# google-research/frame-interpolation

Measured on NVIDIA H100. Metric: interpolated_frames_per_sec_1080p, higher is better.
Workload: dtype f16x2-split (activations/weights as fp16 hi+lo planes; fp32 accumulate)

## Files before the change

### frame_interpolation_b200/csrc/film_conv3x3_tc.cu

```cuda
#include <cuda.h>
#include <cuda_runtime.h>
#include <stdint.h>

#include <type_traits>

#include "film_conv.h"
#include "film_tc_ptx.cuh"

namespace film {
namespace {
using namespace tc;

constexpr int kConsumers = 256;
constexpr int kThreads = kConsumers + 128;
__host__ __device__ constexpr int a_plane_bytes(int kc, int th, int tw) { return (th + 2) * tw * kc * 2; }
__host__ __device__ constexpr int a_stage_bytes(int kc, int th, int tw) { return 2 * a_plane_bytes(kc, th, tw); }
constexpr int kHaloW = 10;
__host__ __device__ constexpr int halo_box_bytes(int kc, int th) { return (th + 2) * kHaloW * kc * 2; }
__host__ __device__ constexpr int halo_plane_bytes(int kc, int th) { return (halo_box_bytes(kc, th) + 1023) & ~1023; }
__host__ __device__ constexpr int a_stage_bytes_h(int kc, int th, int tw, int halo, int planes = 2) {
  return planes * (halo ? halo_plane_bytes(kc, th) : a_plane_bytes(kc, th, tw));
}
constexpr int kMaxRing = 8;
constexpr int kSmemLimit = 227 * 1024;
constexpr int kBarBytes = 8 * (4 * kMaxRing + 4);
constexpr int kFixedBytes = kBarBytes + 16 + 512 * 4  + 64  + 1024  + 64;
constexpr int kHeadW3 = 64 * 32 * 4, kHeadMisc = 512;
constexpr int kHeadBytes = kHeadW3 + kHeadMisc;
constexpr int kPxnStageWg = 64 * 64 * 2;
constexpr int kPxnStageBytes = 2 * kPxnStageWg;
inline int epi_scratch_bytes(int epi_mode, int pxn) { return epi_mode == 3 ? kHeadBytes : pxn ? kPxnStageBytes : 0; }

__host__ __device__ inline int w_tap_bytes(int bn, int kc, int planes = 2) { return bn * kc * 2 * planes; }

template <int BN, int KC, bool kPartial, bool kHalo, bool kOne, bool kRes, bool kPxN = false>
__global__ void __launch_bounds__(kThreads, 1) k_conv3x3_tc(const ConvProblem* __restrict__ prob) {
  static_assert(!kPxN || ((BN == 64 || BN == 128) && KC == 64), "pixels on N: one or two M = 64 weight tiles, 64-channel chunks");
  extern __shared__ uint8_t smem_raw[];
  constexpr bool one = kOne;
  const int planes = one ? 1 : 2;
  constexpr int kWPlane = BN * KC * 2;
  const int kWTap = kWPlane * planes;
  const int kTileH = prob->tile_h, kTileW = prob->tile_w;
  constexpr int kHaloTileH = kPxN ? 32 : 16;
  constexpr int kHaloBox = halo_box_bytes(KC, kHaloTileH), kHaloPlane = halo_plane_bytes(KC, kHaloTileH);
  constexpr bool halo = kHalo;
  const int kAPlane = halo ? kHaloPlane : a_plane_bytes(KC, kTileH, kTileW);
  const int kAStage = planes * kAPlane;
  const int kRowStep = kTileW * KC * 2;
  constexpr bool kFused = BN <= 128 && !kPxN;
  constexpr int kMh = kPxN ? BN / 64 : 1;
  constexpr int kAccRegs = kPxN ? 64 * kMh : (kFused ? 2 * BN : BN) / 2;
  constexpr int kWgPx = kPxN ? 128 : 64;

  const int NA = prob->v2_na, NW = prob->v2_nw;
  const bool resident = prob->v2_resident != 0;
  const int nsrc = prob->nsrc;
  const int tiles_x = prob->tiles_x, tiles_per_img = prob->tiles_y * prob->tiles_x;
  const int cout = prob->cout;
  const int n_nt = (cout + BN - 1) / BN;
  const int ntiles = prob->B * tiles_per_img * n_nt;
  constexpr int kStageTaps = kHalo ? 9 : 3;
  constexpr bool kPacked = kPartial && kPxN;
  const int part_lo = prob->v2_part_lo, part_hi = prob->v2_part_hi;
  int nab = 0;
  for (int s = 0; s < nsrc; ++s) nab += prob->src[s].nchunk * (kHalo ? 1 : 3);
  const int nkb = nab * kStageTaps - (kPacked ? (part_hi - part_lo) * (kStageTaps - kStageTaps / 3) : 0);

  const FastDiv div_nt(n_nt, ntiles), div_img(tiles_per_img, ntiles), div_tx(tiles_x, ntiles);
  const bool pair = prob->pair != 0;
  const int rank = pair ? (int)cluster_ctarank() : 0;
  const int nsp = prob->B * tiles_per_img;
  const int nwork = pair ? ((nsp + 1) / 2) * n_nt : ntiles;
  const int w_first = pair ? (int)blockIdx.x >> 1 : (int)blockIdx.x, w_step = pair ? (int)gridDim.x >> 1 : (int)gridDim.x;
  auto decode = [&](int work, int& sp, int& nti) {
    div_nt.divmod(work, sp, nti);
    if (pair) sp = 2 * sp + rank;
  };

  const uint32_t raw = smem_u32(smem_raw);
  const uint32_t base = (raw + 1023u) & ~1023u;
  uint8_t* gen_base = smem_raw + (base - raw);
// ... 83 lines not shown
        for (int ch = 0; ch < nchunk; ++ch) {
          const int nst = halo ? 1 : 3;
          for (int dx = 0; dx < nst; ++dx, ++ab) {
            const int st = ra.stage;
            mbar_wait(tail + 8u * (kMaxRing + st), ra.phase ^ 1u);
            if (elect_one()) {
              const uint32_t sa = a_base + st * kAStage, bar = tail + 8u * st;
              mbar_expect_tx(bar, halo ? (uint32_t)(planes * kHaloBox) : (uint32_t)kAStage);
              tma_load_4d(sa, tm_hi, bar, c_off + ch * KC, x0 + dx - 1, y0 - 1, bs);
              if (!one) tma_load_4d(sa + kAPlane, tm_lo, bar, c_off + ch * KC, x0 + dx - 1, y0 - 1, bs);
            }
            __syncwarp();
            ra.advance(NA);
            if (!resident) {
              const bool packed = kPacked && ab >= part_lo && ab < part_hi;
              const int nblk = packed ? kStageTaps / 3 : kStageTaps;
              for (int t = 0; t < nblk; ++t, ++kb) {
                const int ws = rw.stage;
                mbar_wait(tail + 8u * (3 * kMaxRing + ws), rw.phase ^ 1u);
                if (elect_one()) {
                  const uint32_t sw = w_base + ws * kWTap, bar = tail + 8u * (2 * kMaxRing + ws);
                  mbar_expect_tx(bar, kWTap);
                  if (pair) {
                    const uint32_t hoff = (uint32_t)(rank * (kWPlane / 2));
                    tma_load_2d_mc(sw + hoff, &prob->tm_w_hi_half, bar, kb * KC, n0 + rank * (BN / 2), 3);
                    if (!one) tma_load_2d_mc(sw + kWPlane + hoff, &prob->tm_w_lo_half, bar, kb * KC, n0 + rank * (BN / 2), 3);
                  } else {
                    tma_load_2d(sw, tm_w_hi, bar, kb * KC, n0);
                    if (!one) tma_load_2d(sw + kWPlane, tm_w_lo, bar, kb * KC, n0);
                  }
                }
// ... 45 lines not shown

  if (resident) mbar_wait(tail + 8u * (2 * kMaxRing), 0);
  const bool is_leader = (threadIdx.x & 127) == 0;
  const uint32_t w_empty_peer = pair ? map_to_cta(tail + 8u * (3 * kMaxRing), (uint32_t)(rank ^ 1)) : 0u;
  auto release_w = [&](int slot) {
    mbar_arrive(tail + 8u * (3 * kMaxRing + slot));
    if (pair) mbar_arrive_cluster(w_empty_peer + 8u * slot);
  };
  {
    constexpr int kWTapC = kWPlane * (kOne ? 1 : 2);
    constexpr uint32_t kPx = KC * 2;
    const uint32_t a_row0 = kHalo ? (uint32_t)(wg * (kWgPx / 8) * kHaloW) * kPx : (uint32_t)(wg * kWgPx) * kPx;
    const uint32_t sbo = kHalo ? kHaloW * kPx : 8 * kPx;
    RingPos ra, rw;
    float acc[kAccRegs];
    auto pxn_mma = [&](uint64_t w_hi, uint64_t w_lo, uint64_t a_hi, uint64_t a_lo, uint32_t accf) {
#pragma unroll
      for (int h = 0; h < kMh; ++h) {
        const uint64_t wh = (uint64_t)(h * (64 * KC * 2) >> 4);
        wgmma<128>(acc + 64 * h, w_hi + wh, a_hi, accf);
        if constexpr (!kOne) {
          wgmma<128>(acc + 64 * h, w_lo + wh, a_hi, 1u);
          wgmma<128>(acc + 64 * h, w_hi + wh, a_lo, 1u);
        }
      }
    };
    for (int tile = w_first; tile < nwork; tile += w_step) {
      int kb = 0;
      int rel_a = -1, rel_w = -1;
      auto retire = [&](int next_a, int next_w) {
        wgmma_commit();
        wgmma_wait<1>();
        if (is_leader) {
          if (rel_a >= 0) mbar_arrive(tail + 8u * (kMaxRing + rel_a));
          if (rel_w >= 0) release_w(rel_w);
        }
        rel_a = next_a;
        rel_w = next_w;
      };
      auto stage = [&](auto ksteps_c, auto tpb_c) {
        constexpr int kSteps = decltype(ksteps_c)::value, kTpb = decltype(tpb_c)::value;
        constexpr int kBlocks = kStageTaps / kTpb;
        const int st = ra.stage;
        mbar_wait(tail + 8u * st, ra.phase);
        const uint32_t sa = a_base + st * kAStage + a_row0;
        const uint32_t lo_off = (uint32_t)(kHalo ? kHaloPlane : kAPlane);
        if constexpr (kRes) {
          const uint64_t a0 = make_desc_sbo<KC>(sa, sbo);
          const uint64_t lo_delta = (uint64_t)(lo_off >> 4);
          const uint64_t row_delta = (uint64_t)(kRowStep >> 4);
          const uint64_t w0 = make_desc_kc<KC>(w_base + kb * kWTapC);
          const uint32_t first = (kb == 0) ? 0u : 1u;
          wgmma_fence();
#pragma unroll
          for (int t = 0; t < kStageTaps; ++t) {
            const uint64_t a_hi = a0 + (kHalo ? (uint64_t)((((t % 3) * kHaloW + t / 3) * kPx) >> 4) : (uint64_t)t * row_delta);
            const uint64_t a_lo = a_hi + lo_delta;
            const uint64_t w_hi = w0 + (uint64_t)(((t / kTpb) * kWTapC + (t % kTpb) * kSteps * 32) >> 4);
            const uint64_t w_lo = w_hi + (uint64_t)(kWPlane >> 4);
#pragma unroll
            for (int k = 0; k < kSteps; ++k) {
              const uint64_t adv = (uint64_t)(k * 32 >> 4);
              const uint32_t accf = (t == 0 && k == 0) ? first : 1u;
              if constexpr (kPxN) {
                pxn_mma(w_hi + adv, w_lo + adv, a_hi + adv, a_lo + adv, accf);
              } else if constexpr (kOne) {
                wgmma<BN>(acc, a_hi + adv, w_hi + adv, accf);
              } else if constexpr (kFused) {
                wgmma<BN>(acc, a_hi + adv, w_hi + adv, accf);
                wgmma<BN>(acc + BN / 2, a_hi + adv, w_lo + adv, accf);
                wgmma<BN>(acc, a_lo + adv, w_hi + adv, 1u);
              } else {
                wgmma<BN>(acc, a_lo + adv, w_hi + adv, accf);
                wgmma<BN>(acc, a_hi + adv, w_lo + adv, 1u);
                wgmma<BN>(acc, a_hi + adv, w_hi + adv, 1u);
              }
            }
          }
// ... 2 lines not shown
        } else {
          for (int blk = 0; blk < kBlocks; ++blk, ++kb) {
            uint32_t sw;
            int ws = -1;
            if (resident) {
              sw = w_base + kb * kWTap;
            } else {
              ws = rw.stage;
              mbar_wait(tail + 8u * (2 * kMaxRing + ws), rw.phase);
              sw = w_base + ws * kWTap;
            }
            const uint32_t first = (kb == 0) ? 0u : 1u;
            wgmma_fence();
#pragma unroll
            for (int u = 0; u < kTpb; ++u) {
              const int t = blk * kTpb + u;
              const uint32_t off = kHalo ? (uint32_t)((t % 3) * kHaloW + t / 3) * kPx : (uint32_t)(t * kRowStep);
              const uint64_t a_hi = make_desc_sbo<KC>(sa + off, sbo);
              const uint64_t a_lo = make_desc_sbo<KC>(sa + lo_off + off, sbo);
              const uint64_t wk = (uint64_t)((u * kSteps * 32) >> 4);
              const uint64_t w_hi = make_desc_kc<KC>(sw) + wk, w_lo = make_desc_kc<KC>(sw + kWPlane) + wk;
#pragma unroll
              for (int k = 0; k < kSteps; ++k) {
                const uint64_t adv = (uint64_t)(k * 32 >> 4);
                const uint32_t accf = (u == 0 && k == 0) ? first : 1u;
                if constexpr (kPxN) {
                  pxn_mma(w_hi + adv, w_lo + adv, a_hi + adv, a_lo + adv, accf);
                } else if constexpr (kOne) {
                  wgmma<BN>(acc, a_hi + adv, w_hi + adv, accf);
                } else if constexpr (kFused) {
                  wgmma<BN>(acc, a_hi + adv, w_hi + adv, accf);
// ... 22 lines not shown
        for (int ab = 0; ab < nab; ++ab) stage(Full{}, One{});
      }
      wgmma_wait<0>();
      if (is_leader) {
        if (rel_a >= 0) mbar_arrive(tail + 8u * (kMaxRing + rel_a));
        if (rel_w >= 0) release_w(rel_w);
      }
      acc_fence<kAccRegs>(acc);

      int sp, nti, b, rem, ty, tx;
      decode(tile, sp, nti);
      div_img.divmod(sp, b, rem);
      div_tx.divmod(rem, ty, tx);
      const int n0 = nti * BN;
      const bool live = sp < nsp;
      if constexpr (kPxN) {
        const int c0 = 16 * (warp & 3) + (lane >> 2);
#pragma unroll
        for (int m = 0; m < kMh; ++m) {
          const float bias0 = bias_smem[n0 + 64 * m + c0], bias1 = bias_smem[n0 + 64 * m + c0 + 8];
#pragma unroll
          for (int i = 64 * m; i < 64 * m + 64; ++i) {
            const float f = acc[i] + ((i & 2) ? bias1 : bias0);
            acc[i] = act ? leaky(f) : f;
          }
        }
        const int y_wg = ty * kTileH + 16 * wg, x_t = tx * kTileW;
        if (do_pool) {
          const int px = x_t + 2 * q;
#pragma unroll
          for (int j = 0; j < 16; j += 2) {
// ... 189 lines not shown
            uint32_t hi, lo;
            split_pack2((a[0][0] + a[1][0]) * 0.25f, (a[0][1] + a[1][1]) * 0.25f, hi, lo);
            *reinterpret_cast<uint32_t*>(pool_hi + ppix * pool_C + n0 + c) = hi;
            *reinterpret_cast<uint32_t*>(pool_lo + ppix * pool_C + n0 + c) = lo;
          }
        }
      }
    }
  }
  leave();
}

int smem_bytes_for(const ConvProblem& h, int bn) {
  const int nkb = h.ktot / h.kchunk;
  const int planes = h.passes == 1 ? 1 : 2;
  const int w = h.v2_resident ? nkb * w_tap_bytes(bn, h.kchunk, planes) : h.v2_nw * w_tap_bytes(bn, h.kchunk, planes);
  return h.v2_na * a_stage_bytes_h(h.kchunk, h.tile_h, h.tile_w, h.halo, planes) + w + kFixedBytes +
         epi_scratch_bytes(h.epi_mode, h.pxn);
}

}

int conv_tc_block_n(int cout);

namespace {
bool ring_depths(int kc, int tile_h, int tile_w, int halo, int planes, int bn, int cout, int ktot, int epi_mode, int pxn,
                 int& resident, int& na, int& nw) {
  const int wtap = w_tap_bytes(bn, kc, planes);
  const int w_all = (ktot / kc) * wtap;
  const int kLimit = kSmemLimit - epi_scratch_bytes(epi_mode, pxn);
  const int kAStage = a_stage_bytes_h(kc, tile_h, tile_w, halo, planes);
  if (cout <= bn && w_all + 2 * kAStage + kFixedBytes <= kLimit) {
    resident = 1;
    const int n = (kLimit - kFixedBytes - w_all) / kAStage;
    const int n_max = halo ? 3 : 6;
    na = n > n_max ? n_max : n;
    nw = 1;
    return true;
  }
  resident = 0;
  na = halo ? 2 : (bn >= 128 ? 2 : 3);
  int n = (kLimit - kFixedBytes - na * kAStage) / wtap;
  if (n < 2 && na > 2) {
    na = 2;
    n = (kLimit - kFixedBytes - na * kAStage) / wtap;
// ... 16 lines not shown
    if (!ring_depths(kc, c[0], c[1], 0, passes == 1 ? 1 : 2, bn, cout, ktot, epi_mode, 0, res, na, nw)) continue;
    const long tiles = (long)B * ((H + c[0] - 1) / c[0]) * ((W + c[1] - 1) / c[1]) * n_nt;
    const long waves = (tiles + num_sms - 1) / num_sms;
    const double cost = (double)waves * (c[0] + 2.0) / c[0] * (1.0 + 1e-3 * (c[1] / 8));
    if (cost < best) {
      best = cost;
      tile_h = c[0];
      tile_w = c[1];
    }
  }
}

bool conv3x3_tc_plan(ConvProblem& h, int num_sms) {
  const int bn = h.bn;
  const int planes = h.passes == 1 ? 1 : 2;
  const int wtap = w_tap_bytes(bn, h.kchunk, planes);
  const int w_all = (h.ktot / h.kchunk) * wtap;
  const bool can_resident = h.cout <= bn;
  const int kLimit = kSmemLimit - epi_scratch_bytes(h.epi_mode, h.pxn);
  if (h.halo && (h.tile_h != (h.pxn ? 32 : 16) || h.tile_w != 8 ||
                 (can_resident && w_all + 2 * a_stage_bytes_h(h.kchunk, h.tile_h, h.tile_w, 0, planes) + kFixedBytes <= kLimit &&
                  w_all + 2 * a_stage_bytes_h(h.kchunk, h.tile_h, h.tile_w, 1, planes) + kFixedBytes > kLimit)))
    h.halo = 0;
  bool ok = ring_depths(h.kchunk, h.tile_h, h.tile_w, h.halo, planes, bn, h.cout, h.ktot, h.epi_mode, h.pxn,
                        h.v2_resident, h.v2_na, h.v2_nw);
  if (!ok && h.halo) {
    h.halo = 0;
    ok = ring_depths(h.kchunk, h.tile_h, h.tile_w, 0, planes, bn, h.cout, h.ktot, h.epi_mode, h.pxn, h.v2_resident,
                     h.v2_na, h.v2_nw);
  }
  const int nsp = h.B * h.tiles_y * h.tiles_x, n_nt = (h.cout + bn - 1) / bn;
  if (h.pair) {
    const int nwork = (nsp + 1) / 2 * n_nt, nclu = num_sms / 2;
    h.v2_grid = 2 * (nwork < nclu ? nwork : nclu);
  } else {
    h.v2_grid = nsp * n_nt < num_sms ? nsp * n_nt : num_sms;
  }
  return ok;
}

template <int BN, int KC, bool kPxN = false>
struct Variants {
  static constexpr void (*kFn[16])(const ConvProblem*) = {
      k_conv3x3_tc<BN, KC, false, false, false, false, kPxN>, k_conv3x3_tc<BN, KC, false, false, false, true, kPxN>,
      k_conv3x3_tc<BN, KC, false, false, true, false, kPxN>,  k_conv3x3_tc<BN, KC, false, false, true, true, kPxN>,
      k_conv3x3_tc<BN, KC, false, true, false, false, kPxN>,  k_conv3x3_tc<BN, KC, false, true, false, true, kPxN>,
      k_conv3x3_tc<BN, KC, false, true, true, false, kPxN>,   k_conv3x3_tc<BN, KC, false, true, true, true, kPxN>,
      k_conv3x3_tc<BN, KC, true, false, false, false, kPxN>,  k_conv3x3_tc<BN, KC, true, false, false, true, kPxN>,
      k_conv3x3_tc<BN, KC, true, false, true, false, kPxN>,   k_conv3x3_tc<BN, KC, true, false, true, true, kPxN>,
      k_conv3x3_tc<BN, KC, true, true, false, false, kPxN>,   k_conv3x3_tc<BN, KC, true, true, false, true, kPxN>,
      k_conv3x3_tc<BN, KC, true, true, true, false, kPxN>,    k_conv3x3_tc<BN, KC, true, true, true, true, kPxN>};
  static cudaError_t configure() {
    for (auto fn : kFn) {
      const cudaError_t e = cudaFuncSetAttribute(fn, cudaFuncAttributeMaxDynamicSharedMemorySize, kSmemLimit);
      if (e != cudaSuccess) return e;
    }
    return cudaSuccess;
  }
  static cudaError_t launch(const ConvProblem* d_prob, const ConvProblem& h, cudaStream_t st) {
    if (h.v2_na < 2 || (!h.v2_resident && h.v2_nw < 2)) return cudaErrorInvalidValue;
    if (kPxN && (h.pair || h.tile_h != 32 || h.tile_w != 8 || h.epi_mode != 0)) return cudaErrorInvalidValue;
    const bool partial = h.v2_part_hi > h.v2_part_lo;
    const int idx = (partial ? 8 : 0) | (h.halo ? 4 : 0) | (h.passes == 1 ? 2 : 0) | (h.v2_resident && h.straight ? 1 : 0);
    if (!h.pair) {
      kFn[idx]<<<h.v2_grid, kThreads, smem_bytes_for(h, BN), st>>>(d_prob);
      return cudaGetLastError();
    }
    cudaLaunchConfig_t cfg = {};
    cudaLaunchAttribute attr[1];
    attr[0].id = cudaLaunchAttributeClusterDimension;
    attr[0].val.clusterDim.x = 2;
    attr[0].val.clusterDim.y = 1;
    attr[0].val.clusterDim.z = 1;
    cfg.gridDim = dim3(h.v2_grid);
    cfg.blockDim = dim3(kThreads);
    cfg.dynamicSmemBytes = smem_bytes_for(h, BN);
    cfg.stream = st;
    cfg.attrs = attr;
// ... 1 lines not shown
    return cudaLaunchKernelEx(&cfg, kFn[idx], d_prob);
  }
};

cudaError_t conv3x3_tc_configure() {
  cudaError_t e;
#define FILM_CFG(BN, KC)                        \
  e = Variants<BN, KC>::configure();            \
  if (e != cudaSuccess) return e;
  FILM_CFG(32, 64) FILM_CFG(64, 64) FILM_CFG(128, 64) FILM_CFG(256, 64) FILM_CFG(32, 32) FILM_CFG(64, 32)
#undef FILM_CFG
  e = Variants<64, 64, true>::configure();
  if (e != cudaSuccess) return e;
  e = Variants<128, 64, true>::configure();
  if (e != cudaSuccess) return e;
  return cudaSuccess;
}

cudaError_t launch_conv3x3_tc(const ConvProblem* d_prob, const ConvProblem& h, cudaStream_t st) {
  const int bn = h.bn;
  if (h.kchunk == 32) {
    if (bn == 32) return Variants<32, 32>::launch(d_prob, h, st);
    if (bn == 64) return Variants<64, 32>::launch(d_prob, h, st);
    return cudaErrorInvalidValue;
  }
  switch (bn) {
    case 256: return Variants<256, 64>::launch(d_prob, h, st);
    case 128: return h.pxn ? Variants<128, 64, true>::launch(d_prob, h, st) : Variants<128, 64>::launch(d_prob, h, st);
    case 64: return h.pxn ? Variants<64, 64, true>::launch(d_prob, h, st) : Variants<64, 64>::launch(d_prob, h, st);
    default: return Variants<32, 64>::launch(d_prob, h, st);
  }
}

}
```

### frame_interpolation_b200/csrc/film_engine.cu

```cuda
#include <cuda.h>
#include <cuda_runtime.h>

#include <algorithm>
#include <cmath>
#include <cstdio>
#include <cstdlib>
#include <cstring>
#include <functional>
#include <map>
#include <memory>
#include <string>
#include <vector>

#include "../../include/film_b200.h"
#include "film_conv.h"
#include "film_kernels.h"
#include "film_pack.h"

namespace film {
int conv_tc_block_n(int cout);

constexpr int kLevels = 7, kFusionLevels = 5, kSpecialized = 3, kSubLevels = 4, kFilters = 64;
static const int kFlowFilters[4] = {32, 64, 128, 256};
static const char* kPredictorNames[4] = {"flow_predictor_0", "flow_predictor_1", "flow_predictor_2",
// ... 253 lines not shown
    FILM_CUDA(cudaMalloc(&d, v.size() * 2));
    allocs.push_back(d);
    FILM_CUDA(cudaMemcpy(d, v.data(), v.size() * 2, cudaMemcpyHostToDevice));
    return d;
  };
  pc.w_hi = upload(hi);
  pc.w_lo = upload(lo);
  pc.pxn_hi = pc.w_hi;
  pc.pxn_lo = pc.w_lo;
  pc.pxn_ktot = ktot;
  std::vector<int> packed;
  for (int ks : pc.src_ksteps) packed.push_back(taps.size() == 9 && chunk == kChunk && ks == 1);
  if (std::count(packed.begin(), packed.end(), 1)) {
    pc.pxn_hi = upload(pack_dx_blocks(hi, cout, ktot, chunk, pc.src_chunks, packed, pc.pxn_ktot));
    pc.pxn_lo = upload(pack_dx_blocks(lo, cout, ktot, chunk, pc.src_chunks, packed, pc.pxn_ktot));
  }
  FILM_CUDA(cudaMalloc(&pc.bias, cout * 4));
  allocs.push_back(pc.bias);
  FILM_CUDA(cudaMemcpy(pc.bias, bias.data.data(), cout * 4, cudaMemcpyHostToDevice));
  return pc;
}

static std::vector<TapSpec> taps_3x3() {
  std::vector<TapSpec> t;
  for (int kx = 0; kx < 3; ++kx)
    for (int ky = 0; ky < 3; ++ky) t.push_back({ky - 1, kx - 1, {{ky, kx}}});
  return t;
}
static std::vector<TapSpec> taps_up2x2(int py, int px) {
  std::vector<TapSpec> t;
// ... 310 lines not shown
  cp.H = s0->H;
  cp.W = s0->W;
  const int kc = pc.kchunk;
  cp.kchunk = kc;
  const bool v2 = o.conv3x3_v2 && o.conv_impl == 0 && pc.ntaps == 9 && (out || epi_mode >= 2) && sy == 1 && sx == 1 &&
                  (kc == kChunk || pc.cout <= 64);
  cp.epi_mode = epi_mode;
  const auto waves = [&](long tiles) { return (tiles + P.num_sms - 1) / P.num_sms; };
  const long pxn_tiles = (long)cp.B * ((cp.H + 31) / 32) * ((cp.W + 7) / 8);
  const long tiles16 = (long)cp.B * ((cp.H + 15) / 16) * ((cp.W + 7) / 8);
  bool skips_ksteps = false;
  for (size_t s = 0; s < pc.src_chunks.size(); ++s)
    if (pc.src_chunks[s] > 0 && pc.src_ksteps[s] != kc / 16) skips_ksteps = true;
  const bool wide = (pc.cout == 128 || pc.cout == 256 || pc.cout == 512) && cp.passes == 1 && !skips_ksteps;
  const bool wide_pays = pc.cout == 128 || (pc.cout == 256 && pc.ktot <= 9 * 1024);
  const long pxn_items = pxn_tiles * (wide ? pc.cout / 128 : 1);
  const bool pxn_pays = skips_ksteps ? 2 * waves(pxn_tiles) <= waves(tiles16)
                                     : pxn_items >= 2L * P.num_sms && (pc.cout == 64 || wide_pays);
  cp.pxn = (v2 && o.conv3x3_pxn && (pc.cout == 64 || wide) && kc == kChunk && epi_mode == 0 && out &&
            out_c_off % 8 == 0 && out->C % 8 == 0 && (!pool_out || pool_out->C % 8 == 0) &&
            (o.conv3x3_pxn >= 2 || pxn_pays)) ? 1 : 0;
  const int ktot = cp.pxn ? pc.pxn_ktot : pc.ktot;
  const sp_t* w_hi = cp.pxn ? pc.pxn_hi : pc.w_hi;
  const sp_t* w_lo = cp.pxn ? pc.pxn_lo : pc.w_lo;
  int box_h, box_w;
  if (v2) {
    if (cp.pxn) {
      cp.tile_h = 32;
      cp.tile_w = 8;
    } else if (pool_out) {
      cp.tile_h = 16;
      cp.tile_w = 8;
    } else {
      conv3x3_tc_pick_tile(cp.H, cp.W, cp.B, pc.cout, kc, cp.passes, ktot, epi_mode, P.num_sms, cp.tile_h, cp.tile_w);
    }
    box_h = cp.tile_h + 2;
// ... 24 lines not shown
    cp.tap_dx[t] = pc.tap_dx[t];
  }
  cp.ktot = ktot;
  cp.w_hi = w_hi;
  cp.w_lo = w_lo;
  cp.bias = pc.bias;
  cp.cout = pc.cout;
  cp.act = act;
  int bn = conv_tc_block_n(pc.cout);
  if (cp.pxn && bn > 128) bn = 128;
  if (out && !pool_out) {
    auto items = [&](int b) { return (long)cp.B * cp.tiles_y * cp.tiles_x * ((pc.cout + b - 1) / b); };
    while (bn > 64 && 2 * items(bn) <= P.num_sms) bn /= 2;
  }
  cp.bn = bn;
  make_w_map(&cp.tm_w_hi, w_hi, pc.cout, ktot, bn, kc);
  make_w_map(&cp.tm_w_lo, w_lo, pc.cout, ktot, bn, kc);
  make_w_map(&cp.tm_w_hi_half, w_hi, pc.cout, ktot, bn / 2, kc);
  make_w_map(&cp.tm_w_lo_half, w_lo, pc.cout, ktot, bn / 2, kc);
  if (out) {
    cp.out_hi = out->hi;
    cp.out_lo = out->lo;
    cp.out_C = out->C;
    cp.out_H = out->H;
    cp.out_W = out->W;
  } else {
    cp.out_C = 0;
    cp.out_H = cp.H;
    cp.out_W = cp.W;
  }
  cp.out_c_off = out_c_off;
  cp.out_sy = sy;
  cp.out_sx = sx;
  cp.out_oy = oy;
// ... 31 lines not shown
    for (int s = 0, ab = 0; s < cp.nsrc; ab += pc.src_chunks[s] * nst, ++s) {
      if (pc.src_chunks[s] == 0 || pc.src_ksteps[s] == kc / 16) continue;
      if (pc.src_ksteps[s] != 1 || cp.v2_part_hi > cp.v2_part_lo)
        throw Error{FILM_ERR_UNSUPPORTED, "persistent 3x3 conv: only one source may skip k-steps, and it must issue one (" +
                                              tag + ")"};
      cp.v2_part_lo = ab;
      cp.v2_part_hi = ab + pc.src_chunks[s] * nst;
    }
  }
  const size_t idx = P.h_probs.size();
  P.h_probs.push_back(cp);
  double k_issued = 0;
  for (size_t si = 0; si < pc.src_chunks.size(); ++si)
    k_issued += (double)pc.src_chunks[si] * pc.ntaps * (v2 ? pc.src_ksteps[si] * 16 : pc.kchunk);
  P.mma_flops += (double)cp.passes * 2.0 * (double)cp.B * cp.tiles_y * cp.tiles_x * (cp.tile_h * cp.tile_w) * k_issued *
                 (double)(((pc.cout + bn - 1) / bn) * bn);
  double alg_bytes = 0;
  {
    const double px = (double)cp.B * cp.H * cp.W, planes_in = cp.passes == 1 ? 1.0 : 2.0;
    for (size_t si = 0; si < pc.src_chunks.size(); ++si) alg_bytes += px * pc.src_chunks[si] * pc.kchunk * 2.0 * planes_in;
    if (out) alg_bytes += px * pc.cout * 2.0 * (cp.out_lo_skip ? 1.0 : 2.0);
    if (pool_out) alg_bytes += px / 4.0 * pc.cout * 4.0;
    if (epi_mode == 2) alg_bytes += px * 12.0;
    if (!out && epi_mode != 2) alg_bytes += px * 24.0;
    alg_bytes += (double)pc.cout * ktot * 2.0 * planes_in;
  }
  P.last_conv_bytes = alg_bytes;
  if (out && sy == 1 && sx == 1 && !tag.empty())
    P.debug["out:" + tag] = DebugTensor{true, out->hi, out->lo, out->pixels(), out->C, out_c_off, pc.cout};
  if (pool_out)
    P.debug["pool:" + tag] = DebugTensor{true, pool_out->hi, pool_out->lo, pool_out->pixels(), pool_out->C, 0, pc.cout};
// ... 1440 lines not shown
```

### frame_interpolation_b200/csrc/film_pack.h

```cpp
#pragma once
#include <stdint.h>

#include <vector>

namespace film {

inline std::vector<uint16_t> pack_dx_blocks(const std::vector<uint16_t>& per_tap, int cout, int ktot, int chunk,
                                            const std::vector<int>& src_chunks, const std::vector<int>& packed,
                                            int& ktot_out) {
  ktot_out = ktot;
  for (size_t s = 0; s < src_chunks.size(); ++s)
    if (packed[s]) ktot_out -= src_chunks[s] * 6 * chunk;
  std::vector<uint16_t> out((size_t)cout * ktot_out, 0);
  for (int n = 0; n < cout; ++n) {
    const uint16_t* src = per_tap.data() + (size_t)n * ktot;
    uint16_t* dst = out.data() + (size_t)n * ktot_out;
    for (size_t s = 0; s < src_chunks.size(); ++s)
      for (int ch = 0; ch < src_chunks[s]; ++ch, src += 9 * chunk) {
        if (!packed[s]) {
          for (int k = 0; k < 9 * chunk; ++k) *dst++ = src[k];
          continue;
        }
        for (int t = 0; t < 9; ++t)
          for (int c = 0; c < 16; ++c) dst[(t / 3) * chunk + (t % 3) * 16 + c] = src[t * chunk + c];
        dst += 3 * chunk;
      }
  }
  return out;
}

}
```

### frame_interpolation_b200/csrc/film_tc_ptx.cuh

```cuda
#pragma once
#include <cuda.h>
#include <cuda_runtime.h>
#include <stdint.h>

#include "film_conv.h"

namespace film {
namespace tc {

__device__ __forceinline__ uint32_t smem_u32(const void* p) {
  return (uint32_t)__cvta_generic_to_shared(p);
}

__device__ __forceinline__ void mbar_init(uint32_t bar, uint32_t count) {
  asm volatile("mbarrier.init.shared::cta.b64 [%0], %1;" ::"r"(bar), "r"(count));
}
__device__ __forceinline__ void mbar_expect_tx(uint32_t bar, uint32_t bytes) {
  asm volatile("mbarrier.arrive.expect_tx.shared::cta.b64 _, [%0], %1;" ::"r"(bar), "r"(bytes)
               : "memory");
}
__device__ __forceinline__ bool mbar_try_wait(uint32_t bar, uint32_t parity) {
  uint32_t ok;
  asm volatile(
      "{\n\t.reg .pred p;\n\t"
// ... 171 lines not shown
      : "+f"(d[0]), "+f"(d[1]), "+f"(d[2]), "+f"(d[3]), "+f"(d[4]), "+f"(d[5]), "+f"(d[6]), "+f"(d[7]), "+f"(d[8]), "+f"(d[9]), "+f"(d[10]), "+f"(d[11]), "+f"(d[12]), "+f"(d[13]), "+f"(d[14]), "+f"(d[15]), "+f"(d[16]), "+f"(d[17]), "+f"(d[18]), "+f"(d[19]), "+f"(d[20]), "+f"(d[21]), "+f"(d[22]), "+f"(d[23]), "+f"(d[24]), "+f"(d[25]), "+f"(d[26]), "+f"(d[27]), "+f"(d[28]), "+f"(d[29]), "+f"(d[30]), "+f"(d[31])
      : "l"(a), "l"(b), "r"(scale_d));
}
template <>
__device__ __forceinline__ void wgmma<128>(float* d, uint64_t a, uint64_t b, uint32_t scale_d) {
  asm volatile(
      "{\n\t.reg .pred p;\n\t"
      "setp.ne.b32 p, %66, 0;\n\t"
      "wgmma.mma_async.sync.aligned.m64n128k16.f32." FILM_WGMMA_AB " "
      "{%0, %1, %2, %3, %4, %5, %6, %7, %8, %9, %10, %11, %12, %13, %14, %15, %16, %17, %18, %19, %20, %21, %22, %23, %24, %25, %26, %27, %28, %29, %30, %31, %32, %33, %34, %35, %36, %37, %38, %39, %40, %41, %42, %43, %44, %45, %46, %47, %48, %49, %50, %51, %52, %53, %54, %55, %56, %57, %58, %59, %60, %61, %62, %63}, "
      "%64, %65, p, 1, 1, 0, 0;\n\t}"
      : "+f"(d[0]), "+f"(d[1]), "+f"(d[2]), "+f"(d[3]), "+f"(d[4]), "+f"(d[5]), "+f"(d[6]), "+f"(d[7]), "+f"(d[8]), "+f"(d[9]), "+f"(d[10]), "+f"(d[11]), "+f"(d[12]), "+f"(d[13]), "+f"(d[14]), "+f"(d[15]), "+f"(d[16]), "+f"(d[17]), "+f"(d[18]), "+f"(d[19]), "+f"(d[20]), "+f"(d[21]), "+f"(d[22]), "+f"(d[23]), "+f"(d[24]), "+f"(d[25]), "+f"(d[26]), "+f"(d[27]), "+f"(d[28]), "+f"(d[29]), "+f"(d[30]), "+f"(d[31]), "+f"(d[32]), "+f"(d[33]), "+f"(d[34]), "+f"(d[35]), "+f"(d[36]), "+f"(d[37]), "+f"(d[38]), "+f"(d[39]), "+f"(d[40]), "+f"(d[41]), "+f"(d[42]), "+f"(d[43]), "+f"(d[44]), "+f"(d[45]), "+f"(d[46]), "+f"(d[47]), "+f"(d[48]), "+f"(d[49]), "+f"(d[50]), "+f"(d[51]), "+f"(d[52]), "+f"(d[53]), "+f"(d[54]), "+f"(d[55]), "+f"(d[56]), "+f"(d[57]), "+f"(d[58]), "+f"(d[59]), "+f"(d[60]), "+f"(d[61]), "+f"(d[62]), "+f"(d[63])
      : "l"(a), "l"(b), "r"(scale_d));
}
template <>
__device__ __forceinline__ void wgmma<256>(float* d, uint64_t a, uint64_t b, uint32_t scale_d) {
  asm volatile(
      "{\n\t.reg .pred p;\n\t"
      "setp.ne.b32 p, %130, 0;\n\t"
      "wgmma.mma_async.sync.aligned.m64n256k16.f32." FILM_WGMMA_AB " "
      "{%0, %1, %2, %3, %4, %5, %6, %7, %8, %9, %10, %11, %12, %13, %14, %15, %16, %17, %18, %19, %20, %21, %22, %23, %24, %25, %26, %27, %28, %29, %30, %31, %32, %33, %34, %35, %36, %37, %38, %39, %40, %41, %42, %43, %44, %45, %46, %47, %48, %49, %50, %51, %52, %53, %54, %55, %56, %57, %58, %59, %60, %61, %62, %63, %64, %65, %66, %67, %68, %69, %70, %71, %72, %73, %74, %75, %76, %77, %78, %79, %80, %81, %82, %83, %84, %85, %86, %87, %88, %89, %90, %91, %92, %93, %94, %95, %96, %97, %98, %99, %100, %101, %102, %103, %104, %105, %106, %107, %108, %109, %110, %111, %112, %113, %114, %115, %116, %117, %118, %119, %120, %121, %122, %123, %124, %125, %126, %127}, "
      "%128, %129, p, 1, 1, 0, 0;\n\t}"
      : "+f"(d[0]), "+f"(d[1]), "+f"(d[2]), "+f"(d[3]), "+f"(d[4]), "+f"(d[5]), "+f"(d[6]), "+f"(d[7]), "+f"(d[8]), "+f"(d[9]), "+f"(d[10]), "+f"(d[11]), "+f"(d[12]), "+f"(d[13]), "+f"(d[14]), "+f"(d[15]), "+f"(d[16]), "+f"(d[17]), "+f"(d[18]), "+f"(d[19]), "+f"(d[20]), "+f"(d[21]), "+f"(d[22]), "+f"(d[23]), "+f"(d[24]), "+f"(d[25]), "+f"(d[26]), "+f"(d[27]), "+f"(d[28]), "+f"(d[29]), "+f"(d[30]), "+f"(d[31]), "+f"(d[32]), "+f"(d[33]), "+f"(d[34]), "+f"(d[35]), "+f"(d[36]), "+f"(d[37]), "+f"(d[38]), "+f"(d[39]), "+f"(d[40]), "+f"(d[41]), "+f"(d[42]), "+f"(d[43]), "+f"(d[44]), "+f"(d[45]), "+f"(d[46]), "+f"(d[47]), "+f"(d[48]), "+f"(d[49]), "+f"(d[50]), "+f"(d[51]), "+f"(d[52]), "+f"(d[53]), "+f"(d[54]), "+f"(d[55]), "+f"(d[56]), "+f"(d[57]), "+f"(d[58]), "+f"(d[59]), "+f"(d[60]), "+f"(d[61]), "+f"(d[62]), "+f"(d[63]), "+f"(d[64]), "+f"(d[65]), "+f"(d[66]), "+f"(d[67]), "+f"(d[68]), "+f"(d[69]), "+f"(d[70]), "+f"(d[71]), "+f"(d[72]), "+f"(d[73]), "+f"(d[74]), "+f"(d[75]), "+f"(d[76]), "+f"(d[77]), "+f"(d[78]), "+f"(d[79]), "+f"(d[80]), "+f"(d[81]), "+f"(d[82]), "+f"(d[83]), "+f"(d[84]), "+f"(d[85]), "+f"(d[86]), "+f"(d[87]), "+f"(d[88]), "+f"(d[89]), "+f"(d[90]), "+f"(d[91]), "+f"(d[92]), "+f"(d[93]), "+f"(d[94]), "+f"(d[95]), "+f"(d[96]), "+f"(d[97]), "+f"(d[98]), "+f"(d[99]), "+f"(d[100]), "+f"(d[101]), "+f"(d[102]), "+f"(d[103]), "+f"(d[104]), "+f"(d[105]), "+f"(d[106]), "+f"(d[107]), "+f"(d[108]), "+f"(d[109]), "+f"(d[110]), "+f"(d[111]), "+f"(d[112]), "+f"(d[113]), "+f"(d[114]), "+f"(d[115]), "+f"(d[116]), "+f"(d[117]), "+f"(d[118]), "+f"(d[119]), "+f"(d[120]), "+f"(d[121]), "+f"(d[122]), "+f"(d[123]), "+f"(d[124]), "+f"(d[125]), "+f"(d[126]), "+f"(d[127])
      : "l"(a), "l"(b), "r"(scale_d));
}

}
}
```

Baseline: 27.38.

## Fold dy tap pairs into M=64 wgmma with N=136 for Cout=32 pixel-on-N convs

Adds a pixels-on-N path for 3x3 convs with 32 output channels. Two vertical taps are packed into one 64-row weight tile, and each MMA uses N=136 so the shifted row's outputs land in extra columns. The two halves are then summed through shared-memory staging in the epilogue. This lets the Cout=32 layers use the M=64 wgmma shape, with six MMAs per nine taps instead of nine half-empty ones. The cost is wasted N columns, extra shared-memory scratch and synchronisation, a new weight-packing routine, and a fused head epilogue on this path.

Measured after the change: 28.55, median of 6. +4.3%, better.

```diff
diff --git a/frame_interpolation_b200/csrc/film_conv3x3_tc.cu b/frame_interpolation_b200/csrc/film_conv3x3_tc.cu
--- a/frame_interpolation_b200/csrc/film_conv3x3_tc.cu
+++ b/frame_interpolation_b200/csrc/film_conv3x3_tc.cu
@@ -29,17 +29,25 @@
 constexpr int kHeadBytes = kHeadW3 + kHeadMisc;
 constexpr int kPxnStageWg = 64 * 64 * 2;
 constexpr int kPxnStageBytes = 2 * kPxnStageWg;
-inline int epi_scratch_bytes(int epi_mode, int pxn) { return epi_mode == 3 ? kHeadBytes : pxn ? kPxnStageBytes : 0; }
-
+constexpr int kFoldLd = 136;
+constexpr int kFoldStageWg = 32 * kFoldLd * 4;
+inline int epi_scratch_bytes(int epi_mode, int pxn, int bn) {
+  if (pxn && bn == 32) return (epi_mode == 3 ? kHeadBytes : 0) + 2 * kFoldStageWg;
+  return epi_mode == 3 ? kHeadBytes : pxn ? kPxnStageBytes : 0;
+}
+
+__host__ __device__ constexpr int w_rows(int bn, int pxn) { return pxn && bn == 32 ? 64 : bn; }
 __host__ __device__ inline int w_tap_bytes(int bn, int kc, int planes = 2) { return bn * kc * 2 * planes; }
 
 template <int BN, int KC, bool kPartial, bool kHalo, bool kOne, bool kRes, bool kPxN = false>
 __global__ void __launch_bounds__(kThreads, 1) k_conv3x3_tc(const ConvProblem* __restrict__ prob) {
-  static_assert(!kPxN || ((BN == 64 || BN == 128) && KC == 64), "pixels on N: one or two M = 64 weight tiles, 64-channel chunks");
+  static_assert(!kPxN || ((BN == 64 || BN == 128) && KC == 64) || (BN == 32 && kOne && !kPartial),
+                "pixels on N: one or two M = 64 weight tiles of 64-channel chunks, or the folded single-pass Cout = 32 form");
   extern __shared__ uint8_t smem_raw[];
   constexpr bool one = kOne;
   const int planes = one ? 1 : 2;
-  constexpr int kWPlane = BN * KC * 2;
+  constexpr bool kFold = kPxN && BN == 32;
+  constexpr int kWPlane = w_rows(BN, kPxN) * KC * 2;
   const int kWTap = kWPlane * planes;
   const int kTileH = prob->tile_h, kTileW = prob->tile_w;
   constexpr int kHaloTileH = kPxN ? 32 : 16;
@@ -49,8 +57,9 @@
   const int kAStage = planes * kAPlane;
   const int kRowStep = kTileW * KC * 2;
   constexpr bool kFused = BN <= 128 && !kPxN;
-  constexpr int kMh = kPxN ? BN / 64 : 1;
-  constexpr int kAccRegs = kPxN ? 64 * kMh : (kFused ? 2 * BN : BN) / 2;
+  constexpr int kMh = kPxN && !kFold ? BN / 64 : 1;
+  constexpr int kPxnN = kFold ? 136 : 128;
+  constexpr int kAccRegs = kPxN ? kPxnN / 2 * kMh : (kFused ? 2 * BN : BN) / 2;
   constexpr int kWgPx = kPxN ? 128 : 64;
 
   const int NA = prob->v2_na, NW = prob->v2_nw;
@@ -61,11 +70,12 @@
   const int n_nt = (cout + BN - 1) / BN;
   const int ntiles = prob->B * tiles_per_img * n_nt;
   constexpr int kStageTaps = kHalo ? 9 : 3;
+  constexpr int kStageMmas = kFold ? 2 * kStageTaps / 3 : kStageTaps;
   constexpr bool kPacked = kPartial && kPxN;
   const int part_lo = prob->v2_part_lo, part_hi = prob->v2_part_hi;
   int nab = 0;
   for (int s = 0; s < nsrc; ++s) nab += prob->src[s].nchunk * (kHalo ? 1 : 3);
-  const int nkb = nab * kStageTaps - (kPacked ? (part_hi - part_lo) * (kStageTaps - kStageTaps / 3) : 0);
+  const int nkb = nab * kStageMmas - (kPacked ? (part_hi - part_lo) * (kStageTaps - kStageTaps / 3) : 0);
 
   const FastDiv div_nt(n_nt, ntiles), div_img(tiles_per_img, ntiles), div_tx(tiles_x, ntiles);
   const bool pair = prob->pair != 0;
@@ -179,7 +189,7 @@
             ra.advance(NA);
             if (!resident) {
               const bool packed = kPacked && ab >= part_lo && ab < part_hi;
-              const int nblk = packed ? kStageTaps / 3 : kStageTaps;
+              const int nblk = packed ? kStageTaps / 3 : kStageMmas;
               for (int t = 0; t < nblk; ++t, ++kb) {
                 const int ws = rw.stage;
                 mbar_wait(tail + 8u * (3 * kMaxRing + ws), rw.phase ^ 1u);
@@ -255,14 +265,15 @@
     const uint32_t sbo = kHalo ? kHaloW * kPx : 8 * kPx;
     RingPos ra, rw;
     float acc[kAccRegs];
+    auto tap_of = [](int m) { return kFold ? (kHalo ? 3 * (m / 2) : 0) + m % 2 : m; };
     auto pxn_mma = [&](uint64_t w_hi, uint64_t w_lo, uint64_t a_hi, uint64_t a_lo, uint32_t accf) {
 #pragma unroll
       for (int h = 0; h < kMh; ++h) {
         const uint64_t wh = (uint64_t)(h * (64 * KC * 2) >> 4);
-        wgmma<128>(acc + 64 * h, w_hi + wh, a_hi, accf);
+        wgmma<kPxnN>(acc + 64 * h, w_hi + wh, a_hi, accf);
         if constexpr (!kOne) {
-          wgmma<128>(acc + 64 * h, w_lo + wh, a_hi, 1u);
-          wgmma<128>(acc + 64 * h, w_hi + wh, a_lo, 1u);
+          wgmma<kPxnN>(acc + 64 * h, w_lo + wh, a_hi, 1u);
+          wgmma<kPxnN>(acc + 64 * h, w_hi + wh, a_lo, 1u);
         }
       }
     };
@@ -281,7 +292,7 @@
       };
       auto stage = [&](auto ksteps_c, auto tpb_c) {
         constexpr int kSteps = decltype(ksteps_c)::value, kTpb = decltype(tpb_c)::value;
-        constexpr int kBlocks = kStageTaps / kTpb;
+        constexpr int kBlocks = kStageMmas / kTpb;
         const int st = ra.stage;
         mbar_wait(tail + 8u * st, ra.phase);
         const uint32_t sa = a_base + st * kAStage + a_row0;
@@ -294,15 +305,16 @@
           const uint32_t first = (kb == 0) ? 0u : 1u;
           wgmma_fence();
 #pragma unroll
-          for (int t = 0; t < kStageTaps; ++t) {
+          for (int mi = 0; mi < kStageMmas; ++mi) {
+            const int t = tap_of(mi);
             const uint64_t a_hi = a0 + (kHalo ? (uint64_t)((((t % 3) * kHaloW + t / 3) * kPx) >> 4) : (uint64_t)t * row_delta);
             const uint64_t a_lo = a_hi + lo_delta;
-            const uint64_t w_hi = w0 + (uint64_t)(((t / kTpb) * kWTapC + (t % kTpb) * kSteps * 32) >> 4);
+            const uint64_t w_hi = w0 + (uint64_t)(((mi / kTpb) * kWTapC + (mi % kTpb) * kSteps * 32) >> 4);
             const uint64_t w_lo = w_hi + (uint64_t)(kWPlane >> 4);
 #pragma unroll
             for (int k = 0; k < kSteps; ++k) {
               const uint64_t adv = (uint64_t)(k * 32 >> 4);
-              const uint32_t accf = (t == 0 && k == 0) ? first : 1u;
+              const uint32_t accf = (mi == 0 && k == 0) ? first : 1u;
               if constexpr (kPxN) {
                 pxn_mma(w_hi + adv, w_lo + adv, a_hi + adv, a_lo + adv, accf);
               } else if constexpr (kOne) {
@@ -335,7 +347,7 @@
             wgmma_fence();
 #pragma unroll
             for (int u = 0; u < kTpb; ++u) {
-              const int t = blk * kTpb + u;
+              const int t = tap_of(blk * kTpb + u);
               const uint32_t off = kHalo ? (uint32_t)((t % 3) * kHaloW + t / 3) * kPx : (uint32_t)(t * kRowStep);
               const uint64_t a_hi = make_desc_sbo<KC>(sa + off, sbo);
               const uint64_t a_lo = make_desc_sbo<KC>(sa + lo_off + off, sbo);
@@ -388,7 +400,89 @@
       div_tx.divmod(rem, ty, tx);
       const int n0 = nti * BN;
       const bool live = sp < nsp;
-      if constexpr (kPxN) {
+      if constexpr (kFold) {
+        float* const stg = reinterpret_cast<float*>(reinterpret_cast<uint8_t*>(src_tab) + 64 + (fhead ? kHeadBytes : 0) +
+                                                    wg * kFoldStageWg);
+        auto wg_sync = [&]() { asm volatile("bar.sync %0, 128;" ::"r"(2 + wg) : "memory"); };
+        const bool lower = (warp & 2) != 0;
+        const int r0 = 16 * (warp & 1) + (lane >> 2);
+        wg_sync();
+        if (!lower) {
+#pragma unroll
+          for (int j = 0; j < 16; ++j)
+#pragma unroll
+            for (int h = 0; h < 2; ++h)
+              *reinterpret_cast<float2*>(stg + (r0 + 8 * h) * kFoldLd + 8 * j + 2 * q) =
+                  make_float2(acc[4 * j + 2 * h], acc[4 * j + 2 * h + 1]);
+        }
+        wg_sync();
+        if (lower) {
+#pragma unroll
+          for (int j = 1; j < 17; ++j)
+#pragma unroll
+            for (int h = 0; h < 2; ++h) {
+              float2* d = reinterpret_cast<float2*>(stg + (r0 + 8 * h) * kFoldLd + 8 * (j - 1) + 2 * q);
+              const float2 v = *d;
+              *d = make_float2(v.x + acc[4 * j + 2 * h], v.y + acc[4 * j + 2 * h + 1]);
+            }
+        }
+        wg_sync();
+        const int p = threadIdx.x & 127;
+        const int py = ty * kTileH + 16 * wg + (p >> 3), px = tx * kTileW + (p & 7);
+        const int64_t opix = ((int64_t)b * out_H + py) * out_W + px;
+        float f[32];
+#pragma unroll
+        for (int c = 0; c < 32; ++c) {
+          const float x = stg[c * kFoldLd + p] + bias_smem[c];
+          f[c] = act ? leaky(x) : x;
+        }
+        if (!live || py >= H || px >= W) {
+        } else if (fhead) {
+          float hp[16];
+#pragma unroll
+          for (int hh = 0; hh < 16; ++hh) hp[hh] = 0.f;
+#pragma unroll
+          for (int c = 0; c < 32; ++c) {
+            const float4* wr = reinterpret_cast<const float4*>(w3s + c * 16);
+#pragma unroll
+            for (int h4 = 0; h4 < 4; ++h4) {
+              const float4 wv = wr[h4];
+              hp[4 * h4] = fmaf(f[c], wv.x, hp[4 * h4]);
+              hp[4 * h4 + 1] = fmaf(f[c], wv.y, hp[4 * h4 + 1]);
+              hp[4 * h4 + 2] = fmaf(f[c], wv.z, hp[4 * h4 + 2]);
+              hp[4 * h4 + 3] = fmaf(f[c], wv.w, hp[4 * h4 + 3]);
+            }
+          }
+          float f0 = hmisc[3 * 16], f1 = hmisc[3 * 16 + 1];
+#pragma unroll
+          for (int hh = 0; hh < 16; ++hh) {
+            const float x = leaky(hp[hh] + hmisc[hh]);
+            f0 = fmaf(x, hmisc[16 + 2 * hh], f0);
+            f1 = fmaf(x, hmisc[16 + 2 * hh + 1], f1);
+          }
+          float2 res = make_float2(f0, f1), tot = res;
+          if (head_vup) {
+            const float2 u = reinterpret_cast<const float2*>(head_vup)[opix];
+            tot.x += u.x;
+            tot.y += u.y;
+          }
+          reinterpret_cast<float2*>(head_res)[opix] = res;
+          reinterpret_cast<float2*>(head_vout)[opix] = tot;
+        } else {
+          sp_t* const oh = out_hi + opix * out_C + out_c_off;
+          sp_t* const ol = out_lo + opix * out_C + out_c_off;
+#pragma unroll
+          for (int k = 0; k < 4; ++k) {
+            uint32_t hi[4], lo[4];
+#pragma unroll
+            for (int i = 0; i < 4; ++i) split_pack2(f[8 * k + 2 * i], f[8 * k + 2 * i + 1], hi[i], lo[i]);
+            *reinterpret_cast<uint4*>(oh + 8 * k) = make_uint4(hi[0], hi[1], hi[2], hi[3]);
+            if (!lo_skip) *reinterpret_cast<uint4*>(ol + 8 * k) = make_uint4(lo[0], lo[1], lo[2], lo[3]);
+          }
+        }
+        continue;
+      }
+      if constexpr (kPxN && !kFold) {
         const int c0 = 16 * (warp & 3) + (lane >> 2);
 #pragma unroll
         for (int m = 0; m < kMh; ++m) {
@@ -608,9 +702,10 @@
 int smem_bytes_for(const ConvProblem& h, int bn) {
   const int nkb = h.ktot / h.kchunk;
   const int planes = h.passes == 1 ? 1 : 2;
-  const int w = h.v2_resident ? nkb * w_tap_bytes(bn, h.kchunk, planes) : h.v2_nw * w_tap_bytes(bn, h.kchunk, planes);
+  const int wtap = w_tap_bytes(w_rows(bn, h.pxn), h.kchunk, planes);
+  const int w = h.v2_resident ? nkb * wtap : h.v2_nw * wtap;
   return h.v2_na * a_stage_bytes_h(h.kchunk, h.tile_h, h.tile_w, h.halo, planes) + w + kFixedBytes +
-         epi_scratch_bytes(h.epi_mode, h.pxn);
+         epi_scratch_bytes(h.epi_mode, h.pxn, bn);
 }
 
 }
@@ -620,9 +715,9 @@
 namespace {
 bool ring_depths(int kc, int tile_h, int tile_w, int halo, int planes, int bn, int cout, int ktot, int epi_mode, int pxn,
                  int& resident, int& na, int& nw) {
-  const int wtap = w_tap_bytes(bn, kc, planes);
+  const int wtap = w_tap_bytes(w_rows(bn, pxn), kc, planes);
   const int w_all = (ktot / kc) * wtap;
-  const int kLimit = kSmemLimit - epi_scratch_bytes(epi_mode, pxn);
+  const int kLimit = kSmemLimit - epi_scratch_bytes(epi_mode, pxn, bn);
   const int kAStage = a_stage_bytes_h(kc, tile_h, tile_w, halo, planes);
   if (cout <= bn && w_all + 2 * kAStage + kFixedBytes <= kLimit) {
     resident = 1;
@@ -669,10 +764,10 @@
 bool conv3x3_tc_plan(ConvProblem& h, int num_sms) {
   const int bn = h.bn;
   const int planes = h.passes == 1 ? 1 : 2;
-  const int wtap = w_tap_bytes(bn, h.kchunk, planes);
+  const int wtap = w_tap_bytes(w_rows(bn, h.pxn), h.kchunk, planes);
   const int w_all = (h.ktot / h.kchunk) * wtap;
   const bool can_resident = h.cout <= bn;
-  const int kLimit = kSmemLimit - epi_scratch_bytes(h.epi_mode, h.pxn);
+  const int kLimit = kSmemLimit - epi_scratch_bytes(h.epi_mode, h.pxn, bn);
   if (h.halo && (h.tile_h != (h.pxn ? 32 : 16) || h.tile_w != 8 ||
                  (can_resident && w_all + 2 * a_stage_bytes_h(h.kchunk, h.tile_h, h.tile_w, 0, planes) + kFixedBytes <= kLimit &&
                   w_all + 2 * a_stage_bytes_h(h.kchunk, h.tile_h, h.tile_w, 1, planes) + kFixedBytes > kLimit)))
@@ -694,19 +789,29 @@
   return ok;
 }
 
+using ConvKernel = void (*)(const ConvProblem*);
+template <int BN, int KC, bool kPartial, bool kHalo, bool kOne, bool kRes, bool kPxN>
+constexpr ConvKernel kernel_of() {
+  if constexpr (kPxN && BN == 32 && (kPartial || !kOne))
+    return nullptr;
+  else
+    return k_conv3x3_tc<BN, KC, kPartial, kHalo, kOne, kRes, kPxN>;
+}
+
 template <int BN, int KC, bool kPxN = false>
 struct Variants {
-  static constexpr void (*kFn[16])(const ConvProblem*) = {
-      k_conv3x3_tc<BN, KC, false, false, false, false, kPxN>, k_conv3x3_tc<BN, KC, false, false, false, true, kPxN>,
-      k_conv3x3_tc<BN, KC, false, false, true, false, kPxN>,  k_conv3x3_tc<BN, KC, false, false, true, true, kPxN>,
-      k_conv3x3_tc<BN, KC, false, true, false, false, kPxN>,  k_conv3x3_tc<BN, KC, false, true, false, true, kPxN>,
-      k_conv3x3_tc<BN, KC, false, true, true, false, kPxN>,   k_conv3x3_tc<BN, KC, false, true, true, true, kPxN>,
-      k_conv3x3_tc<BN, KC, true, false, false, false, kPxN>,  k_conv3x3_tc<BN, KC, true, false, false, true, kPxN>,
-      k_conv3x3_tc<BN, KC, true, false, true, false, kPxN>,   k_conv3x3_tc<BN, KC, true, false, true, true, kPxN>,
-      k_conv3x3_tc<BN, KC, true, true, false, false, kPxN>,   k_conv3x3_tc<BN, KC, true, true, false, true, kPxN>,
-      k_conv3x3_tc<BN, KC, true, true, true, false, kPxN>,    k_conv3x3_tc<BN, KC, true, true, true, true, kPxN>};
+  static constexpr ConvKernel kFn[16] = {
+      kernel_of<BN, KC, false, false, false, false, kPxN>(), kernel_of<BN, KC, false, false, false, true, kPxN>(),
+      kernel_of<BN, KC, false, false, true, false, kPxN>(),  kernel_of<BN, KC, false, false, true, true, kPxN>(),
+      kernel_of<BN, KC, false, true, false, false, kPxN>(),  kernel_of<BN, KC, false, true, false, true, kPxN>(),
+      kernel_of<BN, KC, false, true, true, false, kPxN>(),   kernel_of<BN, KC, false, true, true, true, kPxN>(),
+      kernel_of<BN, KC, true, false, false, false, kPxN>(),  kernel_of<BN, KC, true, false, false, true, kPxN>(),
+      kernel_of<BN, KC, true, false, true, false, kPxN>(),   kernel_of<BN, KC, true, false, true, true, kPxN>(),
+      kernel_of<BN, KC, true, true, false, false, kPxN>(),   kernel_of<BN, KC, true, true, false, true, kPxN>(),
+      kernel_of<BN, KC, true, true, true, false, kPxN>(),    kernel_of<BN, KC, true, true, true, true, kPxN>()};
   static cudaError_t configure() {
     for (auto fn : kFn) {
+      if (!fn) continue;
       const cudaError_t e = cudaFuncSetAttribute(fn, cudaFuncAttributeMaxDynamicSharedMemorySize, kSmemLimit);
       if (e != cudaSuccess) return e;
     }
@@ -714,9 +819,12 @@
   }
   static cudaError_t launch(const ConvProblem* d_prob, const ConvProblem& h, cudaStream_t st) {
     if (h.v2_na < 2 || (!h.v2_resident && h.v2_nw < 2)) return cudaErrorInvalidValue;
-    if (kPxN && (h.pair || h.tile_h != 32 || h.tile_w != 8 || h.epi_mode != 0)) return cudaErrorInvalidValue;
+    if (kPxN && (h.pair || h.tile_h != 32 || h.tile_w != 8 || h.epi_mode != (BN == 32 && h.epi_mode == 3 ? 3 : 0)))
+      return cudaErrorInvalidValue;
+    if (kPxN && BN == 32 && h.pool_hi) return cudaErrorInvalidValue;
     const bool partial = h.v2_part_hi > h.v2_part_lo;
     const int idx = (partial ? 8 : 0) | (h.halo ? 4 : 0) | (h.passes == 1 ? 2 : 0) | (h.v2_resident && h.straight ? 1 : 0);
+    if (!kFn[idx]) return cudaErrorInvalidValue;
     if (!h.pair) {
       kFn[idx]<<<h.v2_grid, kThreads, smem_bytes_for(h, BN), st>>>(d_prob);
       return cudaGetLastError();
@@ -748,13 +856,17 @@
   if (e != cudaSuccess) return e;
   e = Variants<128, 64, true>::configure();
   if (e != cudaSuccess) return e;
+  e = Variants<32, 64, true>::configure();
+  if (e != cudaSuccess) return e;
+  e = Variants<32, 32, true>::configure();
+  if (e != cudaSuccess) return e;
   return cudaSuccess;
 }
 
 cudaError_t launch_conv3x3_tc(const ConvProblem* d_prob, const ConvProblem& h, cudaStream_t st) {
   const int bn = h.bn;
   if (h.kchunk == 32) {
-    if (bn == 32) return Variants<32, 32>::launch(d_prob, h, st);
+    if (bn == 32) return h.pxn ? Variants<32, 32, true>::launch(d_prob, h, st) : Variants<32, 32>::launch(d_prob, h, st);
     if (bn == 64) return Variants<64, 32>::launch(d_prob, h, st);
     return cudaErrorInvalidValue;
   }
@@ -762,8 +874,8 @@
     case 256: return Variants<256, 64>::launch(d_prob, h, st);
     case 128: return h.pxn ? Variants<128, 64, true>::launch(d_prob, h, st) : Variants<128, 64>::launch(d_prob, h, st);
     case 64: return h.pxn ? Variants<64, 64, true>::launch(d_prob, h, st) : Variants<64, 64>::launch(d_prob, h, st);
-    default: return Variants<32, 64>::launch(d_prob, h, st);
-  }
-}
-
-}
+    default: return h.pxn ? Variants<32, 64, true>::launch(d_prob, h, st) : Variants<32, 64>::launch(d_prob, h, st);
+  }
+}
+
+}
diff --git a/frame_interpolation_b200/csrc/film_engine.cu b/frame_interpolation_b200/csrc/film_engine.cu
--- a/frame_interpolation_b200/csrc/film_engine.cu
+++ b/frame_interpolation_b200/csrc/film_engine.cu
@@ -291,6 +291,10 @@
   if (std::count(packed.begin(), packed.end(), 1)) {
     pc.pxn_hi = upload(pack_dx_blocks(hi, cout, ktot, chunk, pc.src_chunks, packed, pc.pxn_ktot));
     pc.pxn_lo = upload(pack_dx_blocks(lo, cout, ktot, chunk, pc.src_chunks, packed, pc.pxn_ktot));
+  } else if (cout == 32 && taps.size() == 9) {
+    pc.pxn_hi = upload(pack_dy_pairs(hi, ktot, chunk));
+    pc.pxn_lo = upload(pack_dy_pairs(lo, ktot, chunk));
+    pc.pxn_ktot = ktot / 9 * 6;
   }
   FILM_CUDA(cudaMalloc(&pc.bias, cout * 4));
   allocs.push_back(pc.bias);
@@ -631,12 +635,14 @@
     if (pc.src_chunks[s] > 0 && pc.src_ksteps[s] != kc / 16) skips_ksteps = true;
   const bool wide = (pc.cout == 128 || pc.cout == 256 || pc.cout == 512) && cp.passes == 1 && !skips_ksteps;
   const bool wide_pays = pc.cout == 128 || (pc.cout == 256 && pc.ktot <= 9 * 1024);
+  const bool fold = pc.cout == 32 && cp.passes == 1 && !skips_ksteps && !pool_out && (epi_mode == 3 || (epi_mode == 0 && out));
   const long pxn_items = pxn_tiles * (wide ? pc.cout / 128 : 1);
   const bool pxn_pays = skips_ksteps ? 2 * waves(pxn_tiles) <= waves(tiles16)
-                                     : pxn_items >= 2L * P.num_sms && (pc.cout == 64 || wide_pays);
-  cp.pxn = (v2 && o.conv3x3_pxn && (pc.cout == 64 || wide) && kc == kChunk && epi_mode == 0 && out &&
-            out_c_off % 8 == 0 && out->C % 8 == 0 && (!pool_out || pool_out->C % 8 == 0) &&
+                                     : pxn_items >= 2L * P.num_sms && (pc.cout == 64 || wide_pays || fold);
+  const bool pxn_store = epi_mode == 0 && out && out_c_off % 8 == 0 && out->C % 8 == 0 && (!pool_out || pool_out->C % 8 == 0);
+  cp.pxn = (v2 && o.conv3x3_pxn && (((pc.cout == 64 || wide) && kc == kChunk && pxn_store) || (fold && (epi_mode == 3 || pxn_store))) &&
             (o.conv3x3_pxn >= 2 || pxn_pays)) ? 1 : 0;
+  const bool folded = cp.pxn && pc.cout == 32;
   const int ktot = cp.pxn ? pc.pxn_ktot : pc.ktot;
   const sp_t* w_hi = cp.pxn ? pc.pxn_hi : pc.w_hi;
   const sp_t* w_lo = cp.pxn ? pc.pxn_lo : pc.w_lo;
@@ -691,10 +697,11 @@
     while (bn > 64 && 2 * items(bn) <= P.num_sms) bn /= 2;
   }
   cp.bn = bn;
-  make_w_map(&cp.tm_w_hi, w_hi, pc.cout, ktot, bn, kc);
-  make_w_map(&cp.tm_w_lo, w_lo, pc.cout, ktot, bn, kc);
-  make_w_map(&cp.tm_w_hi_half, w_hi, pc.cout, ktot, bn / 2, kc);
-  make_w_map(&cp.tm_w_lo_half, w_lo, pc.cout, ktot, bn / 2, kc);
+  const int w_rows = folded ? 64 : pc.cout, w_box = folded ? 64 : bn;
+  make_w_map(&cp.tm_w_hi, w_hi, w_rows, ktot, w_box, kc);
+  make_w_map(&cp.tm_w_lo, w_lo, w_rows, ktot, w_box, kc);
+  make_w_map(&cp.tm_w_hi_half, w_hi, w_rows, ktot, w_box / 2, kc);
+  make_w_map(&cp.tm_w_lo_half, w_lo, w_rows, ktot, w_box / 2, kc);
   if (out) {
     cp.out_hi = out->hi;
     cp.out_lo = out->lo;
@@ -756,7 +763,7 @@
   for (size_t si = 0; si < pc.src_chunks.size(); ++si)
     k_issued += (double)pc.src_chunks[si] * pc.ntaps * (v2 ? pc.src_ksteps[si] * 16 : pc.kchunk);
   P.mma_flops += (double)cp.passes * 2.0 * (double)cp.B * cp.tiles_y * cp.tiles_x * (cp.tile_h * cp.tile_w) * k_issued *
-                 (double)(((pc.cout + bn - 1) / bn) * bn);
+                 (double)(((pc.cout + bn - 1) / bn) * bn) * (folded ? 17.0 / 12.0 : 1.0);
   double alg_bytes = 0;
   {
     const double px = (double)cp.B * cp.H * cp.W, planes_in = cp.passes == 1 ? 1.0 : 2.0;
diff --git a/frame_interpolation_b200/csrc/film_pack.h b/frame_interpolation_b200/csrc/film_pack.h
--- a/frame_interpolation_b200/csrc/film_pack.h
+++ b/frame_interpolation_b200/csrc/film_pack.h
@@ -29,4 +29,20 @@
   return out;
 }
 
+inline std::vector<uint16_t> pack_dy_pairs(const std::vector<uint16_t>& per_tap, int ktot, int chunk) {
+  const int ktot_out = ktot / 9 * 6;
+  std::vector<uint16_t> out((size_t)64 * ktot_out, 0);
+  for (int g = 0; g < ktot / (9 * chunk); ++g)
+    for (int dx = 0; dx < 3; ++dx)
+      for (int n = 0; n < 32; ++n)
+        for (int c = 0; c < chunk; ++c) {
+          const uint16_t* src = per_tap.data() + (size_t)n * ktot + (size_t)(g * 9 + 3 * dx) * chunk + c;
+          uint16_t* dst = out.data() + (size_t)(g * 6 + 2 * dx) * chunk + c;
+          dst[(size_t)n * ktot_out] = src[0];
+          dst[(size_t)(32 + n) * ktot_out] = src[chunk];
+          dst[(size_t)(32 + n) * ktot_out + chunk] = src[2 * chunk];
+        }
+  return out;
 }
+
+}
diff --git a/frame_interpolation_b200/csrc/film_tc_ptx.cuh b/frame_interpolation_b200/csrc/film_tc_ptx.cuh
--- a/frame_interpolation_b200/csrc/film_tc_ptx.cuh
+++ b/frame_interpolation_b200/csrc/film_tc_ptx.cuh
@@ -209,6 +209,17 @@
       : "l"(a), "l"(b), "r"(scale_d));
 }
 template <>
+__device__ __forceinline__ void wgmma<136>(float* d, uint64_t a, uint64_t b, uint32_t scale_d) {
+  asm volatile(
+      "{\n\t.reg .pred p;\n\t"
+      "setp.ne.b32 p, %70, 0;\n\t"
+      "wgmma.mma_async.sync.aligned.m64n136k16.f32." FILM_WGMMA_AB " "
+      "{%0, %1, %2, %3, %4, %5, %6, %7, %8, %9, %10, %11, %12, %13, %14, %15, %16, %17, %18, %19, %20, %21, %22, %23, %24, %25, %26, %27, %28, %29, %30, %31, %32, %33, %34, %35, %36, %37, %38, %39, %40, %41, %42, %43, %44, %45, %46, %47, %48, %49, %50, %51, %52, %53, %54, %55, %56, %57, %58, %59, %60, %61, %62, %63, %64, %65, %66, %67}, "
+      "%68, %69, p, 1, 1, 0, 0;\n\t}"
+      : "+f"(d[0]), "+f"(d[1]), "+f"(d[2]), "+f"(d[3]), "+f"(d[4]), "+f"(d[5]), "+f"(d[6]), "+f"(d[7]), "+f"(d[8]), "+f"(d[9]), "+f"(d[10]), "+f"(d[11]), "+f"(d[12]), "+f"(d[13]), "+f"(d[14]), "+f"(d[15]), "+f"(d[16]), "+f"(d[17]), "+f"(d[18]), "+f"(d[19]), "+f"(d[20]), "+f"(d[21]), "+f"(d[22]), "+f"(d[23]), "+f"(d[24]), "+f"(d[25]), "+f"(d[26]), "+f"(d[27]), "+f"(d[28]), "+f"(d[29]), "+f"(d[30]), "+f"(d[31]), "+f"(d[32]), "+f"(d[33]), "+f"(d[34]), "+f"(d[35]), "+f"(d[36]), "+f"(d[37]), "+f"(d[38]), "+f"(d[39]), "+f"(d[40]), "+f"(d[41]), "+f"(d[42]), "+f"(d[43]), "+f"(d[44]), "+f"(d[45]), "+f"(d[46]), "+f"(d[47]), "+f"(d[48]), "+f"(d[49]), "+f"(d[50]), "+f"(d[51]), "+f"(d[52]), "+f"(d[53]), "+f"(d[54]), "+f"(d[55]), "+f"(d[56]), "+f"(d[57]), "+f"(d[58]), "+f"(d[59]), "+f"(d[60]), "+f"(d[61]), "+f"(d[62]), "+f"(d[63]), "+f"(d[64]), "+f"(d[65]), "+f"(d[66]), "+f"(d[67])
+      : "l"(a), "l"(b), "r"(scale_d));
+}
+template <>
 __device__ __forceinline__ void wgmma<256>(float* d, uint64_t a, uint64_t b, uint32_t scale_d) {
   asm volatile(
       "{\n\t.reg .pred p;\n\t"
```
